# mosesyhc/LCGP

Measured on AMD Instinct MI355X. Metric: NLL+grad evals/sec, higher is better.
Workload: dtype f64; 1 GPU; configs[2]: n=4096 d=6 p=64 q=8 submethod=full, one NLL+gradient evaluation per step; n=4096, d=6, p=64, q=8, parallelism=latent components k -> rank k mod 1, q_local_rank0=8

## Files before the change

### lcgp_amd/csrc/lcgp_hip.hip

```cpp
#include <hip/hip_runtime.h>
#include <stdint.h>
#include <stdio.h>
#include <string.h>
#include <math.h>
#include <type_traits>
#include <vector>

#include "../../include/lcgp_hip.h"
#include "fill_sched.h"

#define LCGP_VERSION 610

namespace {

constexpr int TS = 64;
constexpr int KT = 16;
constexpr int DMAX = 32;
constexpr int DWIDE = 126;

typedef double d4 __attribute__((ext_vector_type(4)));
typedef float f4 __attribute__((ext_vector_type(4)));

thread_local char g_err[256] = "";

// ... 818 lines not shown
#pragma unroll
        for (int e = 0; e < EPT; ++e) reg[e] = src[e];
    } else {
        constexpr int PE = 16 / (int)sizeof(T), NP = EPT / PE;
#pragma unroll
        for (int pc = 0; pc < NP; ++pc)
#pragma unroll
            for (int e = 0; e < PE; ++e) reg[pc * PE + e] = src[pc * (TM / NP) + e];
    }
}

template <typename T, int L, int TM, int NT, int PC = 0>
__device__ __forceinline__ void load_stage_p(const T* __restrict__ P , int ld, int ks,
                                             typename Piece<T>::v (&reg)[TM * KT / NT * (int)sizeof(T) / 16], unsigned voff) {
    constexpr int EPT = TM * KT / NT;
    constexpr int PE = 16 / (int)sizeof(T), NP = EPT / PE;
    const T* base = L == MK ? P + ks : P + (size_t)ks * ld;
    constexpr int STEP = (L == MK ? PE : TM / NP) * (int)sizeof(T);
    if constexpr (PC < NP) {
        gload_piece<PC * STEP>(reg[PC], voff, base);
        load_stage_p<T, L, TM, NT, PC + 1>(P, ld, ks, reg, voff);
    }
}

template <typename T, int L, int TM, int NT>
__device__ __forceinline__ void store_stage_p(T* __restrict__ S, const typename Piece<T>::v (&reg)[TM * KT / NT * (int)sizeof(T) / 16],
                                              int tid) {
    constexpr int EPT = TM * KT / NT;
    constexpr int LD = TM + 16;
    constexpr int PE = 16 / (int)sizeof(T), NP = EPT / PE;
    if (L == MK) {
        constexpr int TPR = KT / EPT;
        const int m = tid / TPR, kk = (tid % TPR) * EPT;
#pragma unroll
        for (int e = 0; e < EPT; ++e) S[(kk + e) * LD + (m ^ lds_swz<T>(kk + e))] = reg[e / PE][e % PE];
    } else {
        constexpr int TPK = TM / EPT;
        const int kq = tid / TPK, j = tid % TPK;
#pragma unroll
        for (int pc = 0; pc < NP; ++pc)
            *(typename Piece<T>::v*)&S[kq * LD + ((j * PE + pc * (TM / NP)) ^ lds_swz<T>(kq))] = reg[pc];
    }
}

constexpr int LDK = KT + 2;
template <int TM, int NT>
__device__ __forceinline__ void store_stage_rows(double* __restrict__ S, const double (&reg)[TM * KT / NT], int tid) {
    constexpr int EPT = TM * KT / NT, TPR = KT / EPT;
    typedef double d2 __attribute__((ext_vector_type(2)));
    const int m = tid / TPR, kk = (tid % TPR) * EPT;
#pragma unroll
    for (int pc = 0; pc < EPT / 2; ++pc) *(d2*)&S[m * LDK + kk + 2 * pc] = d2{reg[2 * pc], reg[2 * pc + 1]};
}
template <int TM, int NT>
__device__ __forceinline__ void store_stage_rows_p(double* __restrict__ S, const Piece<double>::v (&reg)[TM * KT / NT / 2], int tid) {
    constexpr int EPT = TM * KT / NT, TPR = KT / EPT;
    const int m = tid / TPR, kk = (tid % TPR) * EPT;
#pragma unroll
    for (int pc = 0; pc < EPT / 2; ++pc) *(Piece<double>::v*)&S[m * LDK + kk + 2 * pc] = reg[pc];
}

__device__ __forceinline__ int xcd_remap(int bid, int nwg) {
    const int q = nwg >> 3, r = nwg & 7, x = bid & 7, i = bid >> 3;
    return (x < r ? x * (q + 1) : r * (q + 1) + (x - r) * q) + i;
}

constexpr int VR_DC = 16;
template <typename T, int KERN, int TM, int MIM, int MIN, typename Acc>
__device__ __forceinline__ void vr_epilogue(const GemmArgs& g, const Acc (&acc)[MIM][MIN], int k, int rt, int ct, int tid, int wm0,
                                            int wn0, unsigned char* lds) {
    static_assert(TM == 64 && MIM == 2 && MIN == 2, "the OP_VR epilogue is written for the 64x64 tile on four waves");
    constexpr int XL = VR_DC + 1;
    double* xa = (double*)lds;
    double* xb = xa + TM * XL;
    double* wr = xb + TM * XL;
    double* red = wr + TM;
    static_assert((2 * TM * XL + 2 * TM) * sizeof(double) <= 4 * KT * (TM + 16) * sizeof(T), "fits the stage buffers");
    const int lane = tid & 63, l15 = lane & 15, wave = tid >> 6;
    const int d = g.d;
    const double* th = g.theta + (size_t)k * g.tw;
    const double scale = th[d], nug = th[d + 1], D = th[d + 2];
    const double coff = scale * (1.0 - nug / (1.0 + nug));
    const T* xra = (const T*)g.xa;
    const T* xrb = (const T*)g.xb;
    const int t0 = rt * TM, c0 = ct * TM;
    __syncthreads();
    if (tid < TM) wr[tid] = t0 + tid < g.p2 ? g.wref[t0 + tid] : 0.0;
    double s[MIN];
#pragma unroll
    for (int ni = 0; ni < MIN; ++ni) s[ni] = 0.0;
    const int nch = (d + VR_DC - 1) / VR_DC;
#pragma unroll
    for (int mi = 0; mi < MIM; ++mi)
#pragma unroll
        for (int ni = 0; ni < MIN; ++ni) {
            double pl[4], ss[4];
#pragma unroll
            for (int e = 0; e < 4; ++e) { pl[e] = 1.0; ss[e] = 0.0; }
#pragma unroll 1
            for (int ch = 0; ch < nch; ++ch) {
                const int d0 = ch * VR_DC, dc = d - d0 < VR_DC ? d - d0 : VR_DC;
                if (nch > 1 || (mi == 0 && ni == 0)) {
                    if (ch > 0 || mi > 0 || ni > 0) __syncthreads();
#pragma unroll 1
                    for (int e = tid; e < TM * VR_DC; e += 256) {
                        const int i = e / VR_DC, j = e - i * VR_DC;
                        const int ta = t0 + i, cb = c0 + i;
                        xa[i * XL + j] = (j < dc && ta < g.p2) ? (double)xra[(size_t)ta * d + d0 + j] / th[d0 + j] : 0.0;
                        xb[i * XL + j] = (j < dc && cb < g.p3) ? (double)xrb[(size_t)cb * d + d0 + j] / th[d0 + j] : 0.0;
                    }
                    __syncthreads();
                }
                const double* pa = xa + (wm0 + mi * 16) * XL;
                const double* pb = xb + (wn0 + ni * 16 + l15) * XL;
#pragma unroll 1
                for (int jj = 0; jj < dc; ++jj) {
                    const double yv = pb[jj];
#pragma unroll
                    for (int e = 0; e < 4; ++e) {
                        const double xv = pa[Mfma<T>::row(lane, e) * XL + jj];
                        if constexpr (KERN == 0) {
                            const double sd = fabs(xv - yv);
                            pl[e] = fma(pl[e], sd, pl[e]);
                            ss[e] -= sd;
                        } else if constexpr (KERN == 1) {
                            const double df = xv - yv;
                            ss[e] = fma(-0.5 * df, df, ss[e]);
                        } else {
                            static_assert(KERN == 2, "unknown covariance kernel id");
                            const double sd = fabs(xv - yv);
                            pl[e] = fma(pl[e], m52_fm1(sd), pl[e]);
                            ss[e] -= sd;
                        }
                    }
                }
            }
#pragma unroll
            for (int e = 0; e < 4; ++e) {
                const double c = kern_c0<KERN>(pl[e], ss[e]);
                const double sg = fma(-D, (double)acc[mi][ni][e], coff * c);
                s[ni] = fma(wr[wm0 + mi * 16 + Mfma<T>::row(lane, e)] * sg, sg, s[ni]);
            }
        }
#pragma unroll
    for (int ni = 0; ni < MIN; ++ni) {
        s[ni] += __shfl_xor(s[ni], 16);
        s[ni] += __shfl_xor(s[ni], 32);
    }
    if (wave >= 2 && lane < 16) {
#pragma unroll
        for (int ni = 0; ni < MIN; ++ni) red[wn0 + ni * 16 + l15] = s[ni];
    }
    __syncthreads();
    if (wave < 2 && lane < 16) {
        const double rd = 1.0 / (D * (double)g.nrep);
        double* part = (double*)g.C + ((size_t)k * ((g.p2 + TM - 1) / TM) + rt) * g.ldp;
#pragma unroll
        for (int ni = 0; ni < MIN; ++ni) {
            const int cl = wn0 + ni * 16 + l15, c = c0 + cl;
            if (c < g.p3) part[c] = (s[ni] + red[cl]) / (fmax(g.gvc[(size_t)k * g.ldg + c], 0.0) + rd);
        }
    }
}

template <typename T, int OP, int TM, int NW>
__device__ __forceinline__ void gemm_body(const GemmArgs& g, const int lin ,
                                          unsigned char* lds) {
    constexpr int LA = (OP == OP_LAUUM) ? KM : MK;
    constexpr int LB = (OP == OP_TRTRI_T || OP == OP_TRTRI_W || OP == OP_LAUUM || OP == OP_PRED_V || OP == OP_VG_G || OP == OP_HESS_G) ? KM : MK;
    constexpr int NT = NW * 64;
    constexpr int LD = TM + 16;
    constexpr int WTM = TM / (NW / 2), WTN = TM / 2;
    constexpr int MIM = WTM / 16, MIN = WTN / 16;
    constexpr int EPT = TM * KT / NT;
    T* As = (T*)lds;
    T* Bs = As + 2 * KT * LD;

    int lin_ = lin;
    if constexpr (OP == OP_TRTRI_T || OP == OP_TRTRI_W || OP == OP_LAUUM) {
        if (g.q < 4 && !g.skipq && ((lin >> 8) & 1)) {
            const int base = lin & ~255, nblk = (int)gridDim.x;
            const int top = base + 255 < nblk ? base + 255 : nblk - 1;
            lin_ = top - (lin - base);
        }
    }
    const int k = lin_ % g.q;
    const int bid = lin_ / g.q;
    const T* Ab = (const T*)g.A + (size_t)k * g.sA;
    const T* Bb = (const T*)g.B + (size_t)k * g.sB;
    T* Cb = (T*)g.C + (size_t)k * g.sC;

    const T* A0; const T* B0; T* Ct;
    ptrdiff_t dA, dB;
    int nkt;
    double alpha = 1.0;
    bool accumulate = false;
    bool tri_b = false;
    if constexpr (OP == OP_SYRK) {
        constexpr int SB = 8;
        int t = bid + g.t0, r;
        int i0 = 0;
        for (;;) {
            const int rows = g.nb - g.p2 - i0 < SB ? g.nb - g.p2 - i0 : SB;
            int cnt = 0;
            for (int i = i0; i < i0 + rows; ++i) cnt += (i < g.p3 - g.p2 ? i : g.p3 - g.p2 - 1) + 1;
            if (t < cnt) break;
            t -= cnt;
            i0 += SB;
        }
        const int rows = g.nb - g.p2 - i0 < SB ? g.nb - g.p2 - i0 : SB;
        int j = 0;
        for (;;) {
            const int lo = j > i0 ? j : i0;
            const int cnt = i0 + rows - lo;
            if (t < cnt) { r = g.p2 + lo + t; break; }
            t -= cnt;
            ++j;
        }
        const int c = g.p2 + j;
        A0 = Ab + (size_t)r * TM * g.ldA + (size_t)g.p0 * TM; dA = TM;
        B0 = Bb + (size_t)c * TM * g.ldB + (size_t)g.p0 * TM; dB = TM;
        nkt = g.p1 - g.p0;
        Ct = Cb + (size_t)r * TM * g.ldC + (size_t)c * TM;
        alpha = -1.0; accumulate = true;
    } else if constexpr (OP == OP_TRTRI_T || OP == OP_TRTRI_W) {
        const int mb = g.p0;
        const int npair = g.p1;
        const int pr = g.p2 + bid % npair, rem = bid / npair;
        int rl, cl;
        if constexpr (OP == OP_TRTRI_T) { cl = rem / mb; rl = rem - cl * mb; }
        else { rl = mb - 1 - rem / mb; cl = rem % mb; }
        const int C0 = 2 * pr * mb, R0 = C0 + mb;
        if (R0 + rl >= g.nb) return;
        if constexpr (OP == OP_TRTRI_T) {
            A0 = Ab + (size_t)(R0 + rl) * TM * g.ldA + (size_t)(C0 + mb - 1) * TM; dA = -(ptrdiff_t)TM;
            B0 = Bb + (size_t)(C0 + mb - 1) * TM * g.ldB + (size_t)(C0 + cl) * TM; dB = -(ptrdiff_t)TM * g.ldB;
            nkt = mb - cl;
        } else {
            A0 = Ab + (size_t)(R0 + rl) * TM * g.ldA + (size_t)R0 * TM; dA = TM;
            B0 = Bb + (size_t)R0 * TM * g.ldB + (size_t)(C0 + cl) * TM; dB = (ptrdiff_t)TM * g.ldB;
            nkt = rl + 1;
            alpha = -1.0;
        }
        Ct = Cb + (size_t)(R0 + rl) * TM * g.ldC + (size_t)(C0 + cl) * TM;
    } else if constexpr (OP == OP_LAUUM) {
        int r, c;
        tri_decode(bid, r, c);
        A0 = Ab + (size_t)(g.nb - 1) * TM * g.ldA + (size_t)r * TM; dA = -(ptrdiff_t)TM * g.ldA;
        B0 = Bb + (size_t)(g.nb - 1) * TM * g.ldB + (size_t)c * TM; dB = -(ptrdiff_t)TM * g.ldB;
        nkt = g.nb - r;
        tri_b = r == c;
        Ct = Cb + (size_t)r * TM * g.ldC + (size_t)c * TM;
    } else if constexpr (OP == OP_PRED_COV) {
        int r, c;
        tri_decode(bid, r, c);
        A0 = Ab + (size_t)r * TM * g.ldA; dA = TM;
        B0 = Bb + (size_t)c * TM * g.ldB; dB = TM;
        nkt = g.p0;
        Ct = Cb + (size_t)r * TM * g.ldC + (size_t)c * TM;
        accumulate = true;
    } else if constexpr (OP == OP_VR) {
        const int ct = bid % g.p1, rt = bid / g.p1;
        A0 = Ab + (size_t)rt * TM * g.ldA; dA = TM;
        B0 = Bb + (size_t)ct * TM * g.ldB; dB = TM;
        nkt = g.p0;
        Ct = Cb;
    } else if constexpr (OP == OP_VG_P) {
        const int rt = bid % g.p1, ct = bid / g.p1;
        A0 = Ab + (size_t)ct * TM * g.ldA; dA = TM;
        B0 = Bb + (size_t)rt * TM * g.ldB; dB = TM;
        nkt = g.p0;
        Ct = Cb + (size_t)ct * TM * g.ldC + (size_t)rt * TM;
    } else if constexpr (OP == OP_VG_G || OP == OP_HESS_G) {
        const int c = bid / g.p0, m = bid % g.p0;
        A0 = Ab + (size_t)m * TM * g.ldA; dA = TM;
        B0 = Bb + (size_t)c * TM; dB = (ptrdiff_t)TM * g.ldB;
        nkt = g.p1;
        Ct = Cb + (size_t)m * TM * g.ldC + (size_t)c * TM;
    } else if constexpr (OP == OP_PRED_V) {
        const int c = bid / g.p0, m = bid % g.p0;
        A0 = Ab + (size_t)m * TM * g.ldA + (size_t)(g.nb - 1) * TM; dA = -(ptrdiff_t)TM;
        B0 = Bb + (size_t)(g.nb - 1) * TM * g.ldB + (size_t)c * TM; dB = -(ptrdiff_t)TM * g.ldB;
        nkt = g.nb - c;
        Ct = Cb + (size_t)m * TM * g.ldC + (size_t)c * TM;
    } else {
        const int r = g.nb - 1 - bid / g.p0, m = bid % g.p0;
        A0 = Ab + (size_t)m * TM * g.ldA; dA = TM;
        B0 = Bb + (size_t)r * TM * g.ldB; dB = TM;
        nkt = r + 1;
        Ct = Cb + (size_t)m * TM * g.ldC + (size_t)r * TM;
    }

    const int tid = body_tid();
    const int lane = tid & 63;
    const int wave = __builtin_amdgcn_readfirstlane(tid >> 6);
    const int wm0 = (wave >> 1) * WTM, wn0 = (wave & 1) * WTN;
    typedef typename Mfma<T>::acc_t acc_t;
    acc_t acc[MIM][MIN];
    const __amdgpu_buffer_rsrc_t crs = tile_rsrc(Ct);
    const unsigned cvoff = (unsigned)(Mfma<T>::lane_row(lane) * g.ldC + (lane & 15)) * (unsigned)sizeof(T);
    auto c_soff = [&](int i, int e) -> unsigned {
        return (unsigned)((wm0 + i * 16 + Mfma<T>::reg_row(e)) * g.ldC + wn0) * (unsigned)sizeof(T);
    };
    constexpr bool PRELOAD_C = (OP == OP_SYRK);
#pragma unroll
    for (int i = 0; i < MIM; ++i)
#pragma unroll
        for (int j = 0; j < MIN; ++j)
#pragma unroll
            for (int e = 0; e < 4; ++e) {
                if constexpr (PRELOAD_C) {
                    acc[i][j][e] = BufIo<T>::load(crs, cvoff + j * 16 * (unsigned)sizeof(T), c_soff(i, e));
                } else {
                    acc[i][j][e] = 0;
                }
            }

    constexpr int SPT = TM / KT;
    const int nst = nkt * SPT;
    unsigned long long clk0 = 0, rt0 = 0;
    if constexpr (OP == OP_LAUUM || OP == OP_SYRK) {
        if (g.clk && lin == 0 && wave == 0) { clk0 = __builtin_amdgcn_s_memtime(); rt0 = __builtin_amdgcn_s_memrealtime(); }
    }
    constexpr bool HAS_TRI = OP != OP_SYRK && OP != OP_PRED_COV && OP != OP_VR && OP != OP_VG_P && OP != OP_VG_G && OP != OP_HESS_G;
    const int tri_first = HAS_TRI ? (nkt - 1) * SPT : nst;
    int dead_lo = nst, dead_hi = nst;
    if constexpr (OP == OP_LAUUM) { dead_lo = tri_first; dead_hi = tri_first + (tri_b && wn0 > wm0 ? wn0 : wm0) / KT; }
    else if constexpr (OP == OP_TRTRI_T || OP == OP_PRED_V) { dead_lo = tri_first; dead_hi = tri_first + wn0 / KT; }
    else if constexpr (OP == OP_TRTRI_W) dead_lo = tri_first + (wm0 + WTM) / KT;
    else if constexpr (OP == OP_PRED_U) dead_lo = tri_first + (wn0 + WTN) / KT;
    auto wave_live = [&](int sg) { return !HAS_TRI || sg < dead_lo || sg >= dead_hi; };
    constexpr bool ROWS_A = LA == MK && sizeof(T) == 8, ROWS_B = LB == MK && sizeof(T) == 8;
    static_assert(TM * LDK <= KT * LD, "the row image fits the stage buffer");
    auto put_a = [&](T* S, const T (&reg)[EPT]) {
        if constexpr (ROWS_A) store_stage_rows<TM, NT>((double*)S, (const double (&)[EPT])reg, tid);
        else store_stage<T, LA, TM, NT>(S, reg, tid);
    };
    auto put_b = [&](T* S, const T (&reg)[EPT]) {
        if constexpr (ROWS_B) store_stage_rows<TM, NT>((double*)S, (const double (&)[EPT])reg, tid);
        else store_stage<T, LB, TM, NT>(S, reg, tid);
    };
    auto compute_stage = [&](int buf) {
        const T* as = As + buf * KT * LD;
        const T* bs = Bs + buf * KT * LD;
        const int l15 = lane & 15;
#pragma unroll
        for (int kk = 0; kk < KT / 4; ++kk) {
            const int krow = (kk * 4 + (lane >> 4)) * LD;
            const int kcol = kk * 4 + (lane >> 4);
            T af[MIM], bf[MIN];
#pragma unroll
            for (int i = 0; i < MIM; ++i) {
                const T v = ROWS_A ? as[(wm0 + i * 16 + l15) * LDK + kcol] : as[krow + wm0 + swz_col<T>(i * 16, l15, kk)];
                af[i] = PRELOAD_C ? -v : v;
            }
#pragma unroll
            for (int j = 0; j < MIN; ++j)
                bf[j] = ROWS_B ? bs[(wn0 + j * 16 + l15) * LDK + kcol] : bs[krow + wn0 + swz_col<T>(j * 16, l15, kk)];
#pragma unroll
            for (int i = 0; i < MIM; ++i)
#pragma unroll
                for (int j = 0; j < MIN; ++j) acc[i][j] = Mfma<T>::run(af[i], bf[j], acc[i][j]);
        }
    };
    bool done = false;
    if constexpr (TM == 64) {
        if (nkt == 1) {
            T pa[SPT][EPT], pb[SPT][EPT];
#pragma unroll
            for (int s = 0; s < SPT; ++s) {
                load_stage<T, LA, TM, NT>(A0, g.ldA, s * KT, pa[s], tid);
                load_stage<T, LB, TM, NT>(B0, g.ldB, s * KT, pb[s], tid);
            }
#pragma unroll
            for (int s = 0; s < SPT; ++s) {
                put_a(As + (s & 1) * KT * LD, pa[s]);
                put_b(Bs + (s & 1) * KT * LD, pb[s]);
                __syncthreads();
                if (wave_live(s)) compute_stage(s & 1);
            }
            done = true;
        }
    }
    if (!done) {
        constexpr int PF = OP != OP_SYRK && TM == 64 && sizeof(T) == 4 ? 4 : 2;
        constexpr int NPC = EPT * (int)sizeof(T) / 16;
        constexpr bool COUNTED = PF == 2 && (NPC == 1 || NPC == 2 || NPC == 4) && !PRELOAD_C;
        if constexpr (COUNTED) {
            typedef typename Piece<T>::v pc_t;
            constexpr int NL = 2 * NPC;
            pc_t qa[PF][NPC], qb[PF][NPC];
            auto put_ap = [&](T* S, const pc_t (&reg)[NPC]) {
                if constexpr (ROWS_A) store_stage_rows_p<TM, NT>((double*)S, (const Piece<double>::v (&)[NPC])reg, tid);
                else store_stage_p<T, LA, TM, NT>(S, reg, tid);
            };
            auto put_bp = [&](T* S, const pc_t (&reg)[NPC]) {
                if constexpr (ROWS_B) store_stage_rows_p<TM, NT>((double*)S, (const Piece<double>::v (&)[NPC])reg, tid);
                else store_stage_p<T, LB, TM, NT>(S, reg, tid);
            };
            const unsigned voffA = stage_lane_offset<T, LA, TM, NT>(g.ldA, tid), voffB = stage_lane_offset<T, LB, TM, NT>(g.ldB, tid);
            static_assert(SPT % PF == 0 && SPT >= 2 * PF, "stage count of a k tile");
#pragma unroll
            for (int h = 0; h < PF; ++h) {
                const int kt = h / SPT, ks = (h % SPT) * KT;
                load_stage_p<T, LA, TM, NT>(A0 + (ptrdiff_t)kt * dA, g.ldA, ks, qa[h], voffA);
                load_stage_p<T, LB, TM, NT>(B0 + (ptrdiff_t)kt * dB, g.ldB, ks, qb[h], voffB);
            }
            int s = 0;
            for (; s + 2 * PF <= nst; s += PF) {
#pragma unroll
                for (int h = 0; h < PF; ++h) {
                    const int buf = (PF & 1) ? ((s + h) & 1) : (h & 1);
                    vm_wait_set<(PF - 1) * NL>(qa[h], qb[h]);
                    put_ap(As + buf * KT * LD, qa[h]);
                    put_bp(Bs + buf * KT * LD, qb[h]);
                    __syncthreads();
                    const int kt = (s + h + PF) / SPT, ks = ((s + h + PF) % SPT) * KT;
                    load_stage_p<T, LA, TM, NT>(A0 + (ptrdiff_t)kt * dA, g.ldA, ks, qa[h], voffA);
                    load_stage_p<T, LB, TM, NT>(B0 + (ptrdiff_t)kt * dB, g.ldB, ks, qb[h], voffB);
                    if (wave_live(s + h)) compute_stage(buf);
                }
            }
#pragma unroll
            for (int h = 0; h < PF; ++h) {
                const int buf = (PF & 1) ? ((s + h) & 1) : (h & 1);
                vm_wait_set<0>(qa[h], qb[h]);
                put_ap(As + buf * KT * LD, qa[h]);
                put_bp(Bs + buf * KT * LD, qb[h]);
                __syncthreads();
                if (wave_live(s + h)) compute_stage(buf);
            }
        } else {
            T ra[PF][EPT], rb[PF][EPT];
            const unsigned uoffA = stage_lane_offset<T, LA, TM, NT>(g.ldA, tid), uoffB = stage_lane_offset<T, LB, TM, NT>(g.ldB, tid);
#pragma unroll
            for (int h = 0; h < PF; ++h) {
                if (h < nst) {
                    const int kt = h / SPT, ks = (h % SPT) * KT;
                    load_stage_u<T, LA, TM, NT>(A0 + (ptrdiff_t)kt * dA, g.ldA, ks, ra[h], uoffA);
                    load_stage_u<T, LB, TM, NT>(B0 + (ptrdiff_t)kt * dB, g.ldB, ks, rb[h], uoffB);
                }
            }
            for (int s = 0; s < nst; s += PF) {
#pragma unroll
                for (int h = 0; h < PF; ++h) {
                    if (s + h < nst) {
                        const int buf = (PF & 1) ? ((s + h) & 1) : (h & 1);
                        put_a(As + buf * KT * LD, ra[h]);
                        put_b(Bs + buf * KT * LD, rb[h]);
                        __syncthreads();
                        if (s + h + PF < nst) {
                            const int kt = (s + h + PF) / SPT, ks = ((s + h + PF) % SPT) * KT;
                            load_stage_u<T, LA, TM, NT>(A0 + (ptrdiff_t)kt * dA, g.ldA, ks, ra[h], uoffA);
                            load_stage_u<T, LB, TM, NT>(B0 + (ptrdiff_t)kt * dB, g.ldB, ks, rb[h], uoffB);
                        }
                        if (wave_live(s + h)) compute_stage(buf);
                    }
                }
            }
        }
    }
    if constexpr (OP == OP_VR) {
        const int ct = bid % g.p1, rt = bid / g.p1;
        if (g.kern == 0) vr_epilogue<T, 0, TM, MIM, MIN>(g, acc, k, rt, ct, tid, wm0, wn0, lds);
        else if (g.kern == 1) vr_epilogue<T, 1, TM, MIM, MIN>(g, acc, k, rt, ct, tid, wm0, wn0, lds);
        else vr_epilogue<T, 2, TM, MIM, MIN>(g, acc, k, rt, ct, tid, wm0, wn0, lds);
        return;
    }
    if constexpr (OP == OP_PRED_COV) alpha = -g.theta[(size_t)k * g.p1 + g.p2];
#pragma unroll
    for (int mi = 0; mi < MIM; ++mi)
#pragma unroll
        for (int ni = 0; ni < MIN; ++ni)
#pragma unroll
            for (int e = 0; e < 4; ++e) {
                const unsigned dvoff = cvoff + ni * 16 * (unsigned)sizeof(T), dsoff = c_soff(mi, e);
                if constexpr (OP == OP_SYRK && TM == 128) {
                    if (g.skipq && bid + g.t0 == 0 && wm0 + mi * 16 + Mfma<T>::row(lane, e) < TS && wn0 + ni * 16 + (lane & 15) < TS)
                        continue;
                }
                if constexpr (PRELOAD_C) {
                    BufIo<T>::store((T)acc[mi][ni][e], crs, dvoff, dsoff);
                } else {
                    double v = alpha * (double)acc[mi][ni][e];
                    if (accumulate) v += (double)BufIo<T>::load(crs, dvoff, dsoff);
                    BufIo<T>::store((T)v, crs, dvoff, dsoff);
                }
            }
    if constexpr (OP == OP_LAUUM || OP == OP_SYRK) {
        if (g.clk && lin == 0 && wave == 0) {
            const unsigned long long c1 = __builtin_amdgcn_s_memtime() - clk0, r1 = __builtin_amdgcn_s_memrealtime() - rt0;
            if (lane == 0) { g.clk[0] = c1; g.clk[1] = r1; }
        }
    }
    if constexpr (OP == OP_LAUUM && TM == 128) {
        if (g.part) {
            __syncthreads();
            double* bsh = (double*)lds;
            double* p1s = bsh + 256;
            double* p2s = p1s + 256;
            int r, c;
            tri_decode(bid, r, c);
            const T* bk = (const T*)g.bvec + (size_t)k * g.ldC;
            if (tid < 256) bsh[tid] = (double)bk[(size_t)(tid < 128 ? r : c) * 128 + (tid & 127)];
            __syncthreads();
            const int l15 = lane & 15;
            double s2[MIN];
#pragma unroll
            for (int j = 0; j < MIN; ++j) s2[j] = 0.0;
#pragma unroll
            for (int i = 0; i < MIM; ++i)
#pragma unroll
                for (int e = 0; e < 4; ++e) {
                    const int row = wm0 + i * 16 + Mfma<T>::row(lane, e);
                    const double br = bsh[row];
                    double s1 = 0.0;
#pragma unroll
                    for (int j = 0; j < MIN; ++j) {
                        const double v = (double)acc[i][j][e];
                        s1 = fma(v, bsh[128 + wn0 + j * 16 + l15], s1);
                        s2[j] = fma(v, br, s2[j]);
                    }
                    s1 += __shfl_xor(s1, 1);
                    s1 += __shfl_xor(s1, 2);
                    s1 += __shfl_xor(s1, 4);
                    s1 += __shfl_xor(s1, 8);
                    if (l15 == 0) p1s[(wave & 1) * 128 + row] = s1;
                }
#pragma unroll
            for (int j = 0; j < MIN; ++j) {
                double v = s2[j];
                v += __shfl_xor(v, 16);
                v += __shfl_xor(v, 32);
                if ((lane >> 4) == 0) p2s[(wave >> 1) * 128 + wn0 + j * 16 + l15] = v;
            }
            __syncthreads();
            double* pt = g.part + ((size_t)k * (g.nb * (g.nb + 1) / 2) + bid) * 256;
            if (tid < 128) pt[tid] = p1s[tid] + p1s[128 + tid];
            else if (tid < 256) {
                const int cc = tid - 128;
                pt[128 + cc] = (p2s[cc] + p2s[128 + cc]) + (p2s[256 + cc] + p2s[384 + cc]);
            }
        }
    }
}

template <typename T, int OP, int TM, int NW>
__global__ __launch_bounds__(NW * 64, TM == 128 ? (NW == 8 ? 4 : 2) : (OP == OP_VR ? 2 : 4)) void tile_gemm(GemmArgs g) {
    __shared__ __align__(16) unsigned char lds[4 * KT * (TM + 16) * sizeof(T)];
    gemm_body<T, OP, TM, NW>(g, blockIdx.x, lds);
}

using lcgp_fill::FillJob;
using lcgp_fill::FillSet;

template <typename T, int LA, int LB, bool NEG>
__device__ __forceinline__ void rect_tile(const T* __restrict__ A0, int ldA, const T* __restrict__ B0, int ldB,
                                          T* __restrict__ Ct, int ldC, int nst, bool first, unsigned char* lds) {
    constexpr int TMR = 128, TNC = 64, NT = 256, NJ_ = TNC / 32;
    constexpr int LDA = TMR + 16, LDB = TNC + 16;
    constexpr int EA = TMR * KT / NT, EB = TNC * KT / NT;
    T* As = (T*)lds;
    T* Bs = As + 2 * KT * LDA;
    const int tid = body_tid(), lane = tid & 63, wave = __builtin_amdgcn_readfirstlane(tid >> 6);
    const int wm0 = (wave >> 1) * 64, wn0 = (wave & 1) * (TNC / 2);
    typedef typename Mfma<T>::acc_t acc_t;
    acc_t acc[4][NJ_];
    if (first) {
#pragma unroll
        for (int i = 0; i < 4; ++i)
#pragma unroll
            for (int j = 0; j < NJ_; ++j)
#pragma unroll
                for (int e = 0; e < 4; ++e) acc[i][j][e] = 0;
    } else {
#pragma unroll
        for (int i = 0; i < 4; ++i)
#pragma unroll
            for (int j = 0; j < NJ_; ++j)
#pragma unroll
                for (int e = 0; e < 4; ++e)
                    acc[i][j][e] = Ct[(size_t)(wm0 + i * 16 + Mfma<T>::row(lane, e)) * ldC + wn0 + j * 16 + (lane & 15)];
    }
    T ra[2][EA], rb[2][EB];
    if (nst > 0) {
        load_stage<T, LA, TMR, NT>(A0, ldA, 0, ra[0], tid);
        load_stage<T, LB, TNC, NT>(B0, ldB, 0, rb[0], tid);
    }
    if (nst > 1) {
        load_stage<T, LA, TMR, NT>(A0, ldA, KT, ra[1], tid);
        load_stage<T, LB, TNC, NT>(B0, ldB, KT, rb[1], tid);
    }
    if (nst > 0) {
        store_stage<T, LA, TMR, NT>(As, ra[0], tid);
        store_stage<T, LB, TNC, NT>(Bs, rb[0], tid);
        if (nst > 2) {
            load_stage<T, LA, TMR, NT>(A0, ldA, 2 * KT, ra[0], tid);
            load_stage<T, LB, TNC, NT>(B0, ldB, 2 * KT, rb[0], tid);
        }
        __syncthreads();
    }
    for (int s = 0; s < nst; s += 2) {
#pragma unroll
        for (int h = 0; h < 2; ++h) {
            if (s + h < nst) {
                const T* as = As + h * KT * LDA;
                const T* bs = Bs + h * KT * LDB;
#pragma unroll
                for (int kk = 0; kk < KT / 4; ++kk) {
                    const int kr = kk * 4 + (lane >> 4);
                    T af[4], bf[NJ_];
#pragma unroll
                    for (int i = 0; i < 4; ++i) {
                        const T v = as[kr * LDA + wm0 + swz_col<T>(i * 16, lane & 15, kk)];
                        af[i] = NEG ? -v : v;
                    }
#pragma unroll
                    for (int j = 0; j < NJ_; ++j) bf[j] = bs[kr * LDB + wn0 + swz_col<T>(j * 16, lane & 15, kk)];
#pragma unroll
                    for (int i = 0; i < 4; ++i)
#pragma unroll
                        for (int j = 0; j < NJ_; ++j) acc[i][j] = Mfma<T>::run(af[i], bf[j], acc[i][j]);
                    if (kk == 0 && s + h + 1 < nst) {
                        store_stage<T, LA, TMR, NT>(As + (h ^ 1) * KT * LDA, ra[h ^ 1], tid);
                        store_stage<T, LB, TNC, NT>(Bs + (h ^ 1) * KT * LDB, rb[h ^ 1], tid);
                        if (s + h + 3 < nst) {
                            load_stage<T, LA, TMR, NT>(A0, ldA, (s + h + 3) * KT, ra[h ^ 1], tid);
                            load_stage<T, LB, TNC, NT>(B0, ldB, (s + h + 3) * KT, rb[h ^ 1], tid);
                        }
                    }
                }
                __syncthreads();
            }
        }
    }
#pragma unroll
    for (int i = 0; i < 4; ++i)
#pragma unroll
        for (int j = 0; j < NJ_; ++j)
#pragma unroll
            for (int e = 0; e < 4; ++e)
                Ct[(size_t)(wm0 + i * 16 + Mfma<T>::row(lane, e)) * ldC + wn0 + j * 16 + (lane & 15)] = (T)acc[i][j][e];
}

template <typename T>
__device__ __forceinline__ void fill_dispatch(const FillSet& fs, int b, unsigned char* lds) {
    int ji = 0;
    while (ji + 1 < fs.njobs && b >= fs.job[ji].nblk) { b -= fs.job[ji].nblk; ++ji; }
    const FillJob jb = fs.job[ji];
    const int ld = fs.npad;
    if (jb.type == lcgp_fill::FILL_TRI_T || jb.type == lcgp_fill::FILL_TRI_W) {
        GemmArgs g;
        g.sA = g.sB = g.sC = fs.mat; g.ldA = g.ldB = g.ldC = ld; g.nb = fs.nb;
        g.p0 = jb.R0; g.p1 = jb.R1; g.p2 = jb.j0; g.p3 = 0; g.q = fs.q; g.t0 = 0; g.skipq = 1;
        if (jb.type == lcgp_fill::FILL_TRI_T) {
            g.A = fs.M; g.B = fs.W; g.C = fs.V;
            gemm_body<T, OP_TRTRI_T, 64, 4>(g, b + jb.t0 * fs.q, lds);
        } else {
            g.A = fs.W; g.B = fs.V; g.C = fs.W;
            gemm_body<T, OP_TRTRI_W, 64, 4>(g, b + jb.t0 * fs.q, lds);
        }
        return;
    }
    const int k = b % fs.q;
    int t = b / fs.q + jb.t0;
    T* M = (T*)fs.M + (size_t)k * fs.mat;
    T* W = (T*)fs.W + (size_t)k * fs.mat;
    T* V = (T*)fs.V + (size_t)k * fs.mat;
    const int kb0 = jb.kb0, kb1 = jb.kb1;
    if (jb.type == lcgp_fill::FILL_SYRK) {
        int j = jb.j0;
        while (t >= jb.R1 - (j >> 1)) { t -= jb.R1 - (j >> 1); ++j; }
        const int R = (j >> 1) + t;
        rect_tile<T, MK, MK, true>(M + (size_t)R * 128 * ld + (size_t)kb0 * TS, ld, M + (size_t)j * TS * ld + (size_t)kb0 * TS, ld,
                                   M + (size_t)R * 128 * ld + (size_t)j * TS, ld, (kb1 - kb0) * (TS / KT), false, lds);
    } else if (jb.type == lcgp_fill::FILL_BROW) {
        const int nc = jb.j1 - jb.j0;
        const int R = jb.R0 + t / nc, j = jb.j0 + t % nc;
        const int ke = kb1 < 2 * R + 2 ? kb1 : 2 * R + 2;
        rect_tile<T, MK, KM, true>(W + (size_t)R * 128 * ld + (size_t)kb0 * TS, ld, V + (size_t)kb0 * TS * ld + (size_t)j * TS, ld,
                                   W + (size_t)R * 128 * ld + (size_t)j * TS, ld, (ke - kb0) * (TS / KT), true, lds);
    } else if (jb.type == lcgp_fill::FILL_CUPD) {
        const int nc = jb.j1 - jb.j0;
        const int R = jb.R0 + t / nc, j = jb.j0 + t % nc;
        const bool own = j >= kb0;
        const int ks = kb0 + (own ? ((j - kb0) & ~1) : 0);
        rect_tile<T, MK, KM, false>(M + (size_t)R * 128 * ld + (size_t)ks * TS, ld, W + (size_t)ks * TS * ld + (size_t)j * TS, ld,
                                    V + (size_t)R * 128 * ld + (size_t)j * TS, ld, (kb1 - ks) * (TS / KT), own, lds);
    } else {
        int R = (int)((sqrt(4.0 * (double)t + 1.0) - 1.0) * 0.5);
        while ((R + 1) * (R + 2) <= t) ++R;
        while (R * (R + 1) > t) --R;
        const int j = t - R * (R + 1);
        const bool own = 2 * R >= kb0;
        const int ks = own ? 2 * R : kb0;
        rect_tile<T, KM, KM, false>(W + (size_t)ks * TS * ld + (size_t)R * 128, ld, W + (size_t)ks * TS * ld + (size_t)j * TS, ld,
                                    V + (size_t)R * 128 * ld + (size_t)j * TS, ld, (kb1 - ks) * (TS / KT), own, lds);
    }
}

constexpr int FILL_LDS_BYTES = 2 * KT * (128 + 16 + 64 + 16) * 8;

template <typename T>
__global__ __launch_bounds__(256, 2) void fill_kernel(FillSet fs) {
    __shared__ __align__(16) unsigned char lds[FILL_LDS_BYTES];
    fill_dispatch<T>(fs, blockIdx.x, lds);
}

template <typename T>
__global__ __launch_bounds__(256, 2) void leaf_fill_kernel(T* __restrict__ M, T* __restrict__ W, size_t mat, int npad, int jb,
                                                        double* __restrict__ logdet, int* __restrict__ info,
                                                        int q, FillSet fs) {
    __shared__ __align__(16) unsigned char lds[LEAF_LDS_BYTES];
    if ((int)blockIdx.x < q) leaf_body<T>(lds, blockIdx.x, M, W, mat, npad, jb, logdet, info);
    else fill_dispatch<T>(fs, blockIdx.x - q, lds);
}

struct StepArgs {
    void* M; void* W; size_t mat; int npad; int nb;
    int c, J, pe;
    int diag_end;
    int q;
    int has_special;
    int n_trmm;
    int n_upd;
    int trmm_r0, upd_r0;
    double* logdet; int* info;
    FillSet fs;
};

template <typename T>
struct Tile64 {
    typedef typename Mfma<T>::acc_t acc_t;
    static constexpr int LD = TS + 16, NT = 256, EPT = TS * KT / NT, SPT = TS / KT;
    static __device__ __forceinline__ void load(acc_t (&acc)[2][2], const T* Ct, int ld, int lane, int wm0, int wn0) {
#pragma unroll
        for (int i = 0; i < 2; ++i)
#pragma unroll
            for (int j = 0; j < 2; ++j)
#pragma unroll
                for (int e = 0; e < 4; ++e)
                    acc[i][j][e] = Ct[(size_t)(wm0 + i * 16 + Mfma<T>::row(lane, e)) * ld + wn0 + j * 16 + (lane & 15)];
    }
    static __device__ __forceinline__ void zero(acc_t (&acc)[2][2]) {
#pragma unroll
        for (int i = 0; i < 2; ++i)
#pragma unroll
            for (int j = 0; j < 2; ++j)
#pragma unroll
                for (int e = 0; e < 4; ++e) acc[i][j][e] = 0;
    }
    static __device__ __forceinline__ void store(const acc_t (&acc)[2][2], T* Ct, int ld, int lane, int wm0, int wn0) {
#pragma unroll
        for (int i = 0; i < 2; ++i)
#pragma unroll
            for (int j = 0; j < 2; ++j)
#pragma unroll
                for (int e = 0; e < 4; ++e)
                    Ct[(size_t)(wm0 + i * 16 + Mfma<T>::row(lane, e)) * ld + wn0 + j * 16 + (lane & 15)] = (T)acc[i][j][e];
    }
    static __device__ __forceinline__ void fetch(T (&p)[SPT][EPT], const T* P, int ld, int tid) {
#pragma unroll
        for (int s = 0; s < SPT; ++s) load_stage<T, MK, TS, NT>(P, ld, s * KT, p[s], tid);
    }
    template <bool NEG>
    static __device__ __forceinline__ void mma_regs(acc_t (&acc)[2][2], const T (&pa)[SPT][EPT], const T (&pb)[SPT][EPT],
                                                    T* lds, int tid, int lane, int wm0, int wn0) {
        T* As = lds;
        T* Bs = As + 2 * KT * LD;
#pragma unroll
        for (int s = 0; s < SPT; ++s) {
            store_stage<T, MK, TS, NT>(As + (s & 1) * KT * LD, pa[s], tid);
            store_stage<T, MK, TS, NT>(Bs + (s & 1) * KT * LD, pb[s], tid);
            __syncthreads();
            const T* as = As + (s & 1) * KT * LD;
            const T* bs = Bs + (s & 1) * KT * LD;
#pragma unroll
            for (int kk = 0; kk < KT / 4; ++kk) {
                const int krow = (kk * 4 + (lane >> 4)) * LD;
                T af[2], bf[2];
#pragma unroll
                for (int i = 0; i < 2; ++i) {
                    const T v = as[krow + wm0 + swz_col<T>(i * 16, lane & 15, kk)];
                    af[i] = NEG ? -v : v;
                }
#pragma unroll
                for (int j = 0; j < 2; ++j) bf[j] = bs[krow + wn0 + swz_col<T>(j * 16, lane & 15, kk)];
#pragma unroll
                for (int i = 0; i < 2; ++i)
#pragma unroll
                    for (int j = 0; j < 2; ++j) acc[i][j] = Mfma<T>::run(af[i], bf[j], acc[i][j]);
// ... 3840 lines not shown
```

Before: 95.50 evals/s.

## Defer SYRK C-tile loads into K-loop tail and stream epilogue in chunks

For the f64 SYRK kernel with four waves, the C tile is no longer preloaded into the accumulators before the K loop. Instead, two row-chunks of C are requested during the final K stages and further chunks are requested inside the epilogue, which computes C minus the accumulator. The aim is to cut accumulator register pressure and to hide the C read latency behind the last MFMA stages. In exchange, the epilogue gains a subtraction, C latency may be exposed if the overlap falls short, and the code now relies on the assumption that nst >= 4.

Result: no change. 96.36 evals/s, median of 5 (+0.9%).

```diff
diff --git a/lcgp_amd/csrc/lcgp_hip.hip b/lcgp_amd/csrc/lcgp_hip.hip
--- a/lcgp_amd/csrc/lcgp_hip.hip
+++ b/lcgp_amd/csrc/lcgp_hip.hip
@@ -1144,7 +1144,17 @@
     auto c_soff = [&](int i, int e) -> unsigned {
         return (unsigned)((wm0 + i * 16 + Mfma<T>::reg_row(e)) * g.ldC + wn0) * (unsigned)sizeof(T);
     };
-    constexpr bool PRELOAD_C = (OP == OP_SYRK);
+    auto c_soff_u = [&](int i, int e) -> unsigned { return (unsigned)__builtin_amdgcn_readfirstlane((int)c_soff(i, e)); };
+    constexpr bool LATE_C = OP == OP_SYRK && sizeof(T) == 8 && NW == 4;
+    constexpr bool PRELOAD_C = OP == OP_SYRK && !LATE_C;
+    T cq[2][MIN][4];
+    auto request_c = [&](int i) {
+#pragma unroll
+        for (int j = 0; j < MIN; ++j)
+#pragma unroll
+            for (int e = 0; e < 4; ++e) cq[i & 1][j][e] = BufIo<T>::load(crs, cvoff + j * 16 * (unsigned)sizeof(T), c_soff_u(i, e));
+    };
+    static_assert(!LATE_C || MIM >= 2, "two C chunks are requested inside the K loop");
 #pragma unroll
     for (int i = 0; i < MIM; ++i)
 #pragma unroll
@@ -1219,6 +1229,7 @@
                 put_a(As + (s & 1) * KT * LD, pa[s]);
                 put_b(Bs + (s & 1) * KT * LD, pb[s]);
                 __syncthreads();
+                if constexpr (LATE_C) { if (s < 2) request_c(s); }
                 if (wave_live(s)) compute_stage(s & 1);
             }
             done = true;
@@ -1228,6 +1239,7 @@
         constexpr int PF = OP != OP_SYRK && TM == 64 && sizeof(T) == 4 ? 4 : 2;
         constexpr int NPC = EPT * (int)sizeof(T) / 16;
         constexpr bool COUNTED = PF == 2 && (NPC == 1 || NPC == 2 || NPC == 4) && !PRELOAD_C;
+        static_assert(!LATE_C || COUNTED, "the C chunks are requested by the hand-counted loop");
         if constexpr (COUNTED) {
             typedef typename Piece<T>::v pc_t;
             constexpr int NL = 2 * NPC;
@@ -1249,6 +1261,7 @@
                 load_stage_p<T, LB, TM, NT>(B0 + (ptrdiff_t)kt * dB, g.ldB, ks, qb[h], voffB);
             }
             int s = 0;
+            if constexpr (LATE_C) __builtin_assume(nst >= 2 * PF);
             for (; s + 2 * PF <= nst; s += PF) {
 #pragma unroll
                 for (int h = 0; h < PF; ++h) {
@@ -1266,10 +1279,18 @@
 #pragma unroll
             for (int h = 0; h < PF; ++h) {
                 const int buf = (PF & 1) ? ((s + h) & 1) : (h & 1);
-                vm_wait_set<0>(qa[h], qb[h]);
+                if constexpr (LATE_C) {
+                    if (h == 0) {
+#pragma unroll
+                        for (int hh = 0; hh < PF; ++hh) vm_wait_set<0>(qa[hh], qb[hh]);
+                    }
+                } else {
+                    vm_wait_set<0>(qa[h], qb[h]);
+                }
                 put_ap(As + buf * KT * LD, qa[h]);
                 put_bp(Bs + buf * KT * LD, qb[h]);
                 __syncthreads();
+                if constexpr (LATE_C) { __builtin_amdgcn_sched_barrier(0); request_c(h); __builtin_amdgcn_sched_barrier(0); }
                 if (wave_live(s + h)) compute_stage(buf);
             }
         } else {
@@ -1310,6 +1331,27 @@
         return;
     }
     if constexpr (OP == OP_PRED_COV) alpha = -g.theta[(size_t)k * g.p1 + g.p2];
+    if constexpr (LATE_C) {
+#pragma unroll
+        for (int mi = 0; mi < MIM; ++mi) {
+            T v[MIN][4];
+#pragma unroll
+            for (int ni = 0; ni < MIN; ++ni)
+#pragma unroll
+                for (int e = 0; e < 4; ++e) v[ni][e] = cq[mi & 1][ni][e] - acc[mi][ni][e];
+            if (mi + 2 < MIM) request_c(mi + 2);
+#pragma unroll
+            for (int ni = 0; ni < MIN; ++ni)
+#pragma unroll
+                for (int e = 0; e < 4; ++e) {
+                    if constexpr (TM == 128) {
+                        if (g.skipq && bid + g.t0 == 0 && wm0 + mi * 16 + Mfma<T>::row(lane, e) < TS && wn0 + ni * 16 + (lane & 15) < TS)
+                            continue;
+                    }
+                    BufIo<T>::store(v[ni][e], crs, cvoff + ni * 16 * (unsigned)sizeof(T), c_soff_u(mi, e));
+                }
+        }
+    } else {
 #pragma unroll
     for (int mi = 0; mi < MIM; ++mi)
 #pragma unroll
@@ -1329,6 +1371,7 @@
                     BufIo<T>::store((T)v, crs, dvoff, dsoff);
                 }
             }
+    }
     if constexpr (OP == OP_LAUUM || OP == OP_SYRK) {
         if (g.clk && lin == 0 && wave == 0) {
             const unsigned long long c1 = __builtin_amdgcn_s_memtime() - clk0, r1 = __builtin_amdgcn_s_memrealtime() - rt0;
```
